# pierregab/VUB_Image_denoising

Measured on NVIDIA B200. Metric: denoised_mpix_per_s, higher is better.
Workload: dtype bf16

## Files before the change

vub_image_denoising_b200/csrc/common.cuh:

```cuda
#pragma once

#include <cuda.h>
#include <cuda_runtime.h>
#include <cuda_bf16.h>
#include <cuda_fp16.h>
#include <stdint.h>
#include <stdio.h>
#include <stdarg.h>

#include "../../include/b200dn.h"

namespace b200dn {

void set_error(const char* fmt, ...);
int cuda_fail(cudaError_t e, const char* what);

#define B200DN_CHECK_ARG(cond, ...)                      \
  do {                                                   \
    if (!(cond)) {                                       \
      ::b200dn::set_error(__VA_ARGS__);                  \
      return B200DN_E_ARG;                               \
    }                                                    \
  } while (0)

// ... 59 lines not shown
      : "r"(bar), "r"(parity)
      : "memory");
  return ok;
}
__device__ __forceinline__ bool elect_one() {
  uint32_t pred;
  asm volatile(
      "{\n\t"
      ".reg .pred p;\n\t"
      "elect.sync _|p, 0xffffffff;\n\t"
      "selp.b32 %0, 1, 0, p;\n\t"
      "}"
      : "=r"(pred));
  return pred != 0;
}
#ifndef B200DN_WATCHDOG_CYCLES
#define B200DN_WATCHDOG_CYCLES (4000000000ll)
#endif
__device__ __forceinline__ void mbar_wait(uint32_t bar, uint32_t parity) {
  if (mbar_try_wait(bar, parity)) return;
  const long long t0 = clock64();
  uint32_t spins = 0;
  while (!mbar_try_wait(bar, parity)) {
    if ((++spins & 0x3ff) == 0 && (clock64() - t0) > B200DN_WATCHDOG_CYCLES) {
      printf("b200dn: mbarrier watchdog (block %d thread %d bar 0x%x parity %u)\n", (int)blockIdx.x,
             (int)threadIdx.x, bar, parity);
      __trap();
    }
  }
}

__device__ __forceinline__ void griddep_wait() { asm volatile("griddepcontrol.wait;" ::: "memory"); }
__device__ __forceinline__ void griddep_launch_dependents() { asm volatile("griddepcontrol.launch_dependents;" ::: "memory"); }

__device__ __forceinline__ uint32_t cluster_ctarank() {
  uint32_t r;
  asm volatile("mov.u32 %0, %%cluster_ctarank;" : "=r"(r));
  return r;
}
__device__ __forceinline__ uint32_t mapa_shared(uint32_t addr, uint32_t rank) {
  uint32_t r;
  asm volatile("mapa.shared::cluster.u32 %0, %1, %2;" : "=r"(r) : "r"(addr), "r"(rank));
  return r;
}
__device__ __forceinline__ void mbar_arrive_cluster(uint32_t cluster_addr) {
  asm volatile("mbarrier.arrive.relaxed.cluster.shared::cluster.b64 _, [%0];" ::"r"(cluster_addr) : "memory");
}
__device__ __forceinline__ void mbar_arrive_remote(uint32_t cluster_addr) {
  asm volatile("mbarrier.arrive.shared::cluster.b64 _, [%0];" ::"r"(cluster_addr) : "memory");
}
__device__ __forceinline__ void cluster_sync_all() {
  asm volatile("barrier.cluster.arrive.release.aligned;\n\tbarrier.cluster.wait.acquire.aligned;" ::: "memory");
}

__device__ __forceinline__ void fence_proxy_async_smem() {
  asm volatile("fence.proxy.async.shared::cta;" ::: "memory");
}

__device__ __forceinline__ void tma_prefetch_desc(const void* desc) {
  asm volatile("prefetch.tensormap [%0];" ::"l"(reinterpret_cast<uint64_t>(desc)) : "memory");
}
__device__ __forceinline__ void tma_load_3d(uint32_t dst, const void* desc, uint32_t bar, int c0, int c1, int c2) {
  asm volatile(
      "cp.async.bulk.tensor.3d.shared::cluster.global.mbarrier::complete_tx::bytes [%0], [%1, {%3, %4, %5}], [%2];"
      ::"r"(dst), "l"(reinterpret_cast<uint64_t>(desc)), "r"(bar), "r"(c0), "r"(c1), "r"(c2)
      : "memory");
}
__device__ __forceinline__ void tma_load_4d(uint32_t dst, const void* desc, uint32_t bar, int c0, int c1, int c2,
                                            int c3) {
  asm volatile(
      "cp.async.bulk.tensor.4d.shared::cluster.global.mbarrier::complete_tx::bytes [%0], [%1, {%3, %4, %5, %6}], [%2];"
      ::"r"(dst), "l"(reinterpret_cast<uint64_t>(desc)), "r"(bar), "r"(c0), "r"(c1), "r"(c2), "r"(c3)
      : "memory");
}
__device__ __forceinline__ void tma_load_5d(uint32_t dst, const void* desc, uint32_t bar, int c0, int c1, int c2,
                                            int c3, int c4) {
  asm volatile(
      "cp.async.bulk.tensor.5d.shared::cluster.global.mbarrier::complete_tx::bytes [%0], [%1, {%3, %4, %5, %6, %7}], "
      "[%2];"
      ::"r"(dst), "l"(reinterpret_cast<uint64_t>(desc)), "r"(bar), "r"(c0), "r"(c1), "r"(c2), "r"(c3), "r"(c4)
      : "memory");
}

__device__ __forceinline__ void tma_load_3d_2sm(uint32_t dst, const void* desc, uint32_t bar, int c0, int c1, int c2) {
  asm volatile(
      "cp.async.bulk.tensor.3d.cta_group::2.shared::cluster.global.mbarrier::complete_tx::bytes [%0], [%1, {%3, %4, %5}], "
      "[%2];"
      ::"r"(dst), "l"(reinterpret_cast<uint64_t>(desc)), "r"(bar), "r"(c0), "r"(c1), "r"(c2)
      : "memory");
}
__device__ __forceinline__ void tma_load_4d_2sm(uint32_t dst, const void* desc, uint32_t bar, int c0, int c1, int c2,
                                                int c3) {
  asm volatile(
      "cp.async.bulk.tensor.4d.cta_group::2.shared::cluster.global.mbarrier::complete_tx::bytes [%0], [%1, {%3, %4, %5, "
      "%6}], [%2];"
      ::"r"(dst), "l"(reinterpret_cast<uint64_t>(desc)), "r"(bar), "r"(c0), "r"(c1), "r"(c2), "r"(c3)
      : "memory");
}

__device__ __forceinline__ void tmem_alloc(uint32_t dst_smem, uint32_t ncols) {
  asm volatile("tcgen05.alloc.cta_group::1.sync.aligned.shared::cta.b32 [%0], %1;" ::"r"(dst_smem), "r"(ncols)
               : "memory");
}
__device__ __forceinline__ void tmem_relinquish() {
  asm volatile("tcgen05.relinquish_alloc_permit.cta_group::1.sync.aligned;" ::: "memory");
}
__device__ __forceinline__ void tmem_dealloc(uint32_t taddr, uint32_t ncols) {
  asm volatile("tcgen05.dealloc.cta_group::1.sync.aligned.b32 %0, %1;" ::"r"(taddr), "r"(ncols) : "memory");
}
__device__ __forceinline__ void tc_fence_before() { asm volatile("tcgen05.fence::before_thread_sync;" ::: "memory"); }
__device__ __forceinline__ void tc_fence_after() { asm volatile("tcgen05.fence::after_thread_sync;" ::: "memory"); }
__device__ __forceinline__ void tmem_ld_wait() { asm volatile("tcgen05.wait::ld.sync.aligned;" ::: "memory"); }

__device__ __forceinline__ void umma_f16(uint32_t tmem_d, uint64_t desc_a, uint64_t desc_b, uint32_t idesc,
                                         uint32_t accumulate) {
  asm volatile(
      "{\n\t"
      ".reg .pred p;\n\t"
      "setp.ne.b32 p, %4, 0;\n\t"
      "tcgen05.mma.cta_group::1.kind::f16 [%0], %1, %2, %3, p;\n\t"
      "}"
      ::"r"(tmem_d), "l"(desc_a), "l"(desc_b), "r"(idesc), "r"(accumulate)
      : "memory");
}
__device__ __forceinline__ void umma_commit(uint32_t bar) {
  asm volatile("tcgen05.commit.cta_group::1.mbarrier::arrive::one.shared::cluster.b64 [%0];" ::"r"(bar) : "memory");
}

__device__ __forceinline__ void tmem_alloc_2cta(uint32_t dst_smem, uint32_t ncols) {
  asm volatile("tcgen05.alloc.cta_group::2.sync.aligned.shared::cta.b32 [%0], %1;" ::"r"(dst_smem), "r"(ncols)
               : "memory");
}
__device__ __forceinline__ void tmem_relinquish_2cta() {
  asm volatile("tcgen05.relinquish_alloc_permit.cta_group::2.sync.aligned;" ::: "memory");
}
__device__ __forceinline__ void tmem_dealloc_2cta(uint32_t taddr, uint32_t ncols) {
  asm volatile("tcgen05.dealloc.cta_group::2.sync.aligned.b32 %0, %1;" ::"r"(taddr), "r"(ncols) : "memory");
}
__device__ __forceinline__ void umma_f16_2cta(uint32_t tmem_d, uint64_t desc_a, uint64_t desc_b, uint32_t idesc,
                                              uint32_t accumulate) {
  asm volatile(
      "{\n\t"
      ".reg .pred p;\n\t"
      "setp.ne.b32 p, %4, 0;\n\t"
      "tcgen05.mma.cta_group::2.kind::f16 [%0], %1, %2, %3, p;\n\t"
      "}"
      ::"r"(tmem_d), "l"(desc_a), "l"(desc_b), "r"(idesc), "r"(accumulate)
      : "memory");
}
__device__ __forceinline__ void umma_commit_2cta(uint32_t bar, uint16_t cta_mask) {
  asm volatile("tcgen05.commit.cta_group::2.mbarrier::arrive::one.shared::cluster.multicast::cluster.b64 [%0], %1;"
               ::"r"(bar), "h"(cta_mask)
               : "memory");
}

__device__ __forceinline__ void tmem_ld16(uint32_t taddr, uint32_t (&r)[16]) {
  asm volatile(
      "tcgen05.ld.sync.aligned.32x32b.x16.b32 "
      "{%0, %1, %2, %3, %4, %5, %6, %7, %8, %9, %10, %11, %12, %13, %14, %15}, [%16];"
      : "=r"(r[0]), "=r"(r[1]), "=r"(r[2]), "=r"(r[3]), "=r"(r[4]), "=r"(r[5]), "=r"(r[6]), "=r"(r[7]), "=r"(r[8]),
        "=r"(r[9]), "=r"(r[10]), "=r"(r[11]), "=r"(r[12]), "=r"(r[13]), "=r"(r[14]), "=r"(r[15])
      : "r"(taddr)
      : "memory");
}

__device__ __forceinline__ uint64_t make_sw128_desc(uint32_t smem_addr, uint32_t sbo_bytes) {
// ... 33 lines not shown
```

vub_image_denoising_b200/csrc/igemm_common.cuh:

```cuda
#pragma once
#include "common.cuh"

#include <cudaTypedefs.h>

namespace b200dn {
namespace igemm {

constexpr int BLOCK_M = 128;
constexpr int BLOCK_K = 64;
constexpr int A_BYTES = BLOCK_M * BLOCK_K * 2;
constexpr int MAX_N = 256;
constexpr int NUM_THREADS = 256;
constexpr int EPI_THREADS = 128;
constexpr int MAX_STAGES = 8;

struct __align__(64) KParams {
  CUtensorMap tmA0, tmA1, tmW;
  int taps;
  int B, H, W;
  int n_cblk, last_k16;
  int cout, block_n;
  int mt;
  int n_tiles_per_group, num_n_tiles;
  int tiles_x, tiles_y, num_tiles;
  int n_pairs, pair_a[3], pair_w[3];
  int wgroups;
  int fmt;
  int num_stages, stage_bytes, tmem_cols;
  int slab_w, slab_bytes, num_slabs;
  int slab_tx;
  int wres, n_wplanes;
  int w_taps;
  int cta2, num_m_tiles;
  int epi_staged;
  int up_fold;
  const float* bias;
  const float* slope;
  int out_kind;
  void* out0;
  void* out1;
  int out_ctot, out_coff;
  const void* res0;
  const void* res1;
  int res_ctot;
  float* out_nchw;
  const float* res_nchw;
  int res_bmod;
  int* sat_flag;
#ifdef B200DN_TIMELINE
  unsigned long long* tl;
#endif
};

enum { TL_ENTRY = 0, TL_SETUP = 1, TL_DEP = 2, TL_MMA0 = 3, TL_MMA_END = 4, TL_ACC0 = 5, TL_EPI_END = 6, TL_EXIT = 7, TL_SM = 8 };
#ifdef B200DN_TIMELINE
__device__ __forceinline__ unsigned long long tl_now() {
  unsigned long long t;
  asm volatile("mov.u64 %0, %%globaltimer;" : "=l"(t));
  return t;
}
#define TL_MARK(p, slot)                                          \
  do {                                                            \
    if ((p).tl != nullptr && blockIdx.x == 0) (p).tl[slot] = tl_now(); \
  } while (0)
#define TL_MARK_ONCE(p, slot, flag)                               \
  do {                                                            \
    if (!(flag)) {                                                \
      (flag) = true;                                              \
      TL_MARK(p, slot);                                           \
    }                                                             \
  } while (0)
#else
#define TL_MARK(p, slot) do {} while (0)
#define TL_MARK_ONCE(p, slot, flag) do {} while (0)
#endif

struct TileCoord {
  int b, y0, x0, grp, n0;
};

__device__ __forceinline__ TileCoord decode_tile(int tile, int num_n_tiles, int n_tiles_per_group, int block_n,
                                                 int tiles_x, int tiles_y, int tile_w, int tile_h) {
  TileCoord t;
  const int m_tile = tile / num_n_tiles;
  const int nt = tile - m_tile * num_n_tiles;
  t.grp = nt / n_tiles_per_group;
  t.n0 = (nt - t.grp * n_tiles_per_group) * block_n;
  const int per_img = tiles_x * tiles_y;
  t.b = m_tile / per_img;
  const int r = m_tile - t.b * per_img;
  const int ty = r / tiles_x;
  t.y0 = ty * tile_h;
  t.x0 = (r - ty * tiles_x) * tile_w;
  return t;
}

struct TileWalker {
  int nt, tx, ty, b;
  int s_nt, s_tx, s_ty, s_b;
  int num_n_tiles, tiles_x, tiles_y;
  __device__ __forceinline__ void init(int tile, int stride, int num_n_tiles_, int tiles_x_, int tiles_y_) {
    num_n_tiles = num_n_tiles_, tiles_x = tiles_x_, tiles_y = tiles_y_;
    int m = tile / num_n_tiles;
    nt = tile - m * num_n_tiles;
    int q = m / tiles_x;
    tx = m - q * tiles_x;
    b = q / tiles_y;
    ty = q - b * tiles_y;
    m = stride / num_n_tiles;
    s_nt = stride - m * num_n_tiles;
    q = m / tiles_x;
    s_tx = m - q * tiles_x;
    s_b = q / tiles_y;
    s_ty = q - s_b * tiles_y;
  }
  __device__ __forceinline__ void next() {
    nt += s_nt;
    int c = nt >= num_n_tiles ? 1 : 0;
// ... 470 lines not shown
```

vub_image_denoising_b200/csrc/igemm_sm100.cu:

```cuda
#include "igemm_common.cuh"
#ifdef B200DN_TIMELINE
#include <mutex>
#include <string>
#include <vector>
#endif

#include <mutex>
#include <new>
#include <stdlib.h>
#include <string.h>

#ifndef B200DN_DEFAULT_CONV3X3_IMPL
#define B200DN_DEFAULT_CONV3X3_IMPL 2
#endif

namespace b200dn {

using namespace igemm;

namespace {

constexpr int TILE_W = 16;
constexpr int TILE_H = 8;
constexpr int RING_BYTES = 176 * 1024;
constexpr int TAP_STAGING_BYTES = 32 * 1024;
constexpr int DATA_BYTES = RING_BYTES + TAP_STAGING_BYTES;
constexpr int SMEM_BYTES = 1024 + DATA_BYTES + 256 + 2 * 2 * MAX_N * 4;

template <int MODE, int MT>
constexpr int epi_groups() { return (MODE == 2 && MT == 1) ? 2 : 1; }

template <int MODE, int MT>
__global__ void __launch_bounds__(NUM_THREADS + EPI_THREADS * (epi_groups<MODE, MT>() - 1), 1)
igemm_kernel(const __grid_constant__ KParams p) {
  constexpr int EG = epi_groups<MODE, MT>();
  extern __shared__ uint8_t smem_raw[];
  const uint32_t raw_u32 = smem_u32(smem_raw);
  const uint32_t smem_base = (raw_u32 + 1023u) & ~1023u;
  uint8_t* smem_gen = smem_raw + (smem_base - raw_u32);
  const uint32_t bars = smem_base + DATA_BYTES;
  if (threadIdx.x == 0) TL_MARK(p, TL_ENTRY);
  uint32_t* tmem_ptr_s = reinterpret_cast<uint32_t*>(smem_gen + DATA_BYTES + 160);
  float* epi_bias = reinterpret_cast<float*>(smem_gen + DATA_BYTES + 256);
  float* epi_slope = epi_bias + 2 * MAX_N;

  const int warp = (threadIdx.x >> 5) ^ 4;
  const int lane = threadIdx.x & 31;

  if (warp == 0 && lane == 0) {
    tma_prefetch_desc(&p.tmA0);
    tma_prefetch_desc(&p.tmW);
    if (p.n_pairs > 1) tma_prefetch_desc(&p.tmA1);
  }
  if (warp == 1 && lane == 0) {
    for (int s = 0; s < MAX_STAGES; ++s) {
      mbar_init(bars + s * 8, 2);
      mbar_init(bars + 64 + s * 8, MT);
    }
    for (int a = 0; a < 2; ++a) {
      mbar_init(bars + 128 + a * 8, MT);
      mbar_init(bars + 144 + a * 8, (EPI_THREADS / 32) * EG);
    }
    mbar_fence_init();
  }
  if (warp == 2) {
    tmem_alloc(smem_u32(tmem_ptr_s), static_cast<uint32_t>(p.tmem_cols));
    tmem_relinquish();
  }
  tc_fence_before();
  __syncthreads();
  tc_fence_after();
  const uint32_t tmem_base = *tmem_ptr_s;
  if (threadIdx.x == 0) TL_MARK(p, TL_SETUP);
  griddep_launch_dependents();
  if (warp != 2) griddep_wait();
  if (threadIdx.x == 0) TL_MARK(p, TL_DEP);

  const int num_tiles = p.num_tiles, grid = gridDim.x;
  const int num_n_tiles = p.num_n_tiles, n_tiles_per_group = p.n_tiles_per_group, block_n = p.block_n;
  const int tiles_x = p.tiles_x, tiles_y = p.tiles_y;
  const int n_cblk = p.n_cblk, n_pairs = p.n_pairs, num_stages = p.num_stages, stage_bytes = p.stage_bytes;
  constexpr int KY = MODE == 0 ? 3 : MODE == 1 ? 2 : 1;
  constexpr int KX = KY;
  constexpr uint32_t W_OFF = MT * A_BYTES;
  constexpr int STW = TILE_W * MT;

  if (warp == 0) {
    int stage = 0;
    uint32_t phase = 0;
    const int pa0 = p.pair_a[0], pa1 = p.pair_a[1], pa2 = p.pair_a[2];
    TileWalker tw_;
    tw_.init(blockIdx.x, grid, num_n_tiles, tiles_x, tiles_y);
    for (int tile = blockIdx.x; tile < num_tiles; tile += grid, tw_.next()) {
      const TileCoord t = tw_.coord_groups(block_n, n_tiles_per_group, STW, TILE_H);
      for (int pair = 0; pair < n_pairs; ++pair) {
        const int pa = pair == 0 ? pa0 : pair == 1 ? pa1 : pa2;
        const CUtensorMap* tmA = pa ? &p.tmA1 : &p.tmA0;
#pragma unroll
        for (int ky = 0; ky < KY; ++ky) {
#pragma unroll
          for (int kx = 0; kx < KX; ++kx) {
            for (int cb = 0; cb < n_cblk; ++cb) {
              mbar_wait(bars + 64 + stage * 8, phase ^ 1u);
              if (elect_one()) {
                const uint32_t full = bars + stage * 8;
                const uint32_t a_dst = smem_base + stage * stage_bytes;
                mbar_arrive_expect_tx(full, MT * A_BYTES);
#pragma unroll
                for (int j = 0; j < MT; ++j) {
                  const int xj = t.x0 + j * TILE_W;
                  if (MODE == 0)
                    tma_load_4d(a_dst + j * A_BYTES, tmA, full, cb * BLOCK_K, xj + kx - 1, t.y0 + ky - 1, t.b);
                  else if (MODE == 1)
// ... 22 lines not shown
    tw_.init(blockIdx.x, grid, num_n_tiles, tiles_x, tiles_y);
    for (int tile = blockIdx.x; tile < num_tiles; tile += grid, tw_.next()) {
      const TileCoord t = tw_.coord_groups(block_n, n_tiles_per_group, STW, TILE_H);
      for (int pair = 0; pair < n_pairs; ++pair) {
        const int wbase = pair == 0 ? pw0 : pair == 1 ? pw1 : pw2;
#pragma unroll
        for (int tap = 0; tap < KY * KX; ++tap) {
          const int wslice = wbase + (MODE == 2 ? t.grp : tap);
          for (int cb = 0; cb < n_cblk; ++cb) {
            mbar_wait(bars + 64 + stage * 8, phase ^ 1u);
            if (elect_one()) {
              const uint32_t full = bars + stage * 8;
              mbar_arrive_expect_tx(full, w_bytes);
              tma_load_3d(smem_base + stage * stage_bytes + W_OFF, &p.tmW, full, cb * BLOCK_K, t.n0, wslice);
            }
            __syncwarp();
            if (++stage == num_stages) {
              stage = 0;
              phase ^= 1u;
            }
          }
        }
      }
    }
  } else if (warp == 1 || (warp == 3 && MT == 2)) {
    const int j = warp == 1 ? 0 : 1;
    const uint32_t idesc = make_idesc_f16(static_cast<uint32_t>(p.fmt), static_cast<uint32_t>(block_n));
    const int k_iters = n_pairs * p.taps * n_cblk;
    const int last_k16 = p.last_k16;
    const uint32_t a_off = static_cast<uint32_t>(j * A_BYTES);
    int stage = 0;
    uint32_t phase = 0;
    int local_tile = 0;
    uint32_t ready = 0;
    for (int tile = blockIdx.x; tile < num_tiles; tile += grid, ++local_tile) {
      const int acc = local_tile & 1;
      const uint32_t acc_phase = (local_tile >> 1) & 1;
      mbar_wait(bars + 144 + acc * 8, acc_phase ^ 1u);
      const uint32_t d = tmem_base + static_cast<uint32_t>((acc * MT + j) * block_n);
      uint32_t accumulate = 0;
      int cb = 0;
      for (int kit = 0; kit < k_iters; ++kit) {
        if (!ready) mbar_wait(bars + stage * 8, phase);
        tc_fence_after();
        const uint32_t s_addr = smem_base + stage * stage_bytes;
        const uint32_t empty_bar = bars + 64 + stage * 8;
        const bool full_block = (cb != n_cblk - 1) || (last_k16 == BLOCK_K / 16);
        if (++stage == num_stages) {
          stage = 0;
          phase ^= 1u;
        }
        ready = mbar_test_wait(bars + stage * 8, phase);
        if (elect_one()) {
          const uint64_t adesc = make_sw128_desc(s_addr + a_off, 1024);
          const uint64_t bdesc = make_sw128_desc(s_addr + W_OFF, 1024);
          if (full_block) {
            umma_f16(d, adesc, bdesc, idesc, accumulate);
            umma_f16(d, adesc + 2, bdesc + 2, idesc, 1u);
            umma_f16(d, adesc + 4, bdesc + 4, idesc, 1u);
            umma_f16(d, adesc + 6, bdesc + 6, idesc, 1u);
          } else {
            for (int k = 0; k < last_k16; ++k) umma_f16(d, adesc + 2 * k, bdesc + 2 * k, idesc, k == 0 ? accumulate : 1u);
          }
          umma_commit(empty_bar);
          if (kit == k_iters - 1) umma_commit(bars + 128 + acc * 8);
        }
        __syncwarp();
        accumulate = 1;
        if (++cb == n_cblk) cb = 0;
      }
    }
  } else if (warp >= 4) {
    const int we = warp & 3;
    const int eg = (EG == 2 && warp >= 8) ? 1 : 0;
    const int row = we * 32 + lane;
    const int th = row / TILE_W, tw = row - th * TILE_W;
    const int et = (threadIdx.x & (EPI_THREADS - 1)) + eg * EPI_THREADS;
    const EpiArgs ea = make_epi_args(p);
    const int H = p.H, W = p.W, cout = p.cout;
    const float* bias = p.bias;
    const float* slope = p.slope;
    const bool up = p.wgroups == 4 && MODE == 2;
    const bool staged = p.epi_staged;
    uint8_t* stg = smem_gen + RING_BYTES + (eg * 4 + we) * 4096;
    const int ncols = block_n / EG, col0 = eg * ncols;
    const bool one_n_tile = n_tiles_per_group == 1;
    if (one_n_tile) stage_bias_slope(epi_bias, epi_slope, bias, slope, 0, block_n, cout, et, EPI_THREADS * EG);
    int local_tile = 0;
    uint32_t satm = 0;
    TileWalker tw_;
    tw_.init(blockIdx.x, grid, num_n_tiles, tiles_x, tiles_y);
    for (int tile = blockIdx.x; tile < num_tiles; tile += grid, ++local_tile, tw_.next()) {
      const TileCoord t = tw_.coord_groups(block_n, n_tiles_per_group, STW, TILE_H);
      const int acc = local_tile & 1;
      const uint32_t acc_phase = (local_tile >> 1) & 1;
      float* bs = epi_bias + (one_n_tile ? 0 : acc * MAX_N);
      float* ss = epi_slope + (one_n_tile ? 0 : acc * MAX_N);
      if (!one_n_tile) stage_bias_slope(bs, ss, bias, slope, t.n0, block_n, cout, et, EPI_THREADS * EG);

      mbar_wait(bars + 128 + acc * 8, acc_phase);
      tc_fence_after();

#pragma unroll 1
      for (int j = 0; j < MT; ++j) {
        const int y = t.y0 + th, x = t.x0 + j * TILE_W + tw;
        const bool valid = (y < H) && (x < W);
        const int64_t res_pix = (static_cast<int64_t>(t.b) * H + y) * W + x;
        int64_t out_pix = res_pix;
        if (up) {
          const int ky = t.grp >> 1, kx = t.grp & 1;
          out_pix = (static_cast<int64_t>(t.b) * (2 * H) + (2 * y + ky)) * (2 * W) + (2 * x + kx);
        }
        const uint32_t taddr =
            tmem_base + (static_cast<uint32_t>(we * 32) << 16) + static_cast<uint32_t>((acc * MT + j) * block_n + col0);
        const uint32_t rel = j == MT - 1 ? bars + 144 + acc * 8 : 0u;
        if (MODE == 2 && p.up_fold) {
#pragma unroll 1
          for (int q = 0; q < 4 / EG; ++q) {
            const int ph = eg * (4 / EG) + q, ky = ph >> 1, kx = ph & 1;
            const uint32_t tq = taddr + static_cast<uint32_t>(q * cout);
            const uint32_t relq = q == 4 / EG - 1 ? rel : 0u;
            if (staged) {
              RowMap rm;
              rm.b = t.b, rm.y0 = t.y0, rm.x0 = t.x0 + j * TILE_W, rm.tw_shift = 4, rm.H = H, rm.W = W;
              rm.up = 1, rm.ky = ky, rm.kx = kx;
              epilogue_subtile_staged(ea, tq, cout, bs, ss, rm, we * 32, lane, 0, relq, stg, satm);
            } else {
              const int64_t op = (static_cast<int64_t>(t.b) * (2 * H) + (2 * y + ky)) * (2 * W) + (2 * x + kx);
              epilogue_subtile(ea, tq, cout, bs, ss, valid, t.b, y, x, op, res_pix, 0, relq, satm);
            }
          }
        } else if (staged) {
          RowMap rm;
          rm.b = t.b, rm.y0 = t.y0, rm.x0 = t.x0 + j * TILE_W, rm.tw_shift = 4, rm.H = H, rm.W = W;
          rm.up = up ? 1 : 0, rm.ky = t.grp >> 1, rm.kx = t.grp & 1;
          epilogue_subtile_staged(ea, taddr, ncols, bs + col0, ss + col0, rm, we * 32, lane, t.n0 + col0, rel, stg, satm);
        } else {
          epilogue_subtile(ea, taddr, ncols, bs + col0, ss + col0, valid, t.b, y, x, out_pix, res_pix, t.n0 + col0, rel, satm);
        }
      }
    }
    sat_report(ea.sat_flag, satm);
  }

  tc_fence_before();
  __syncthreads();
  if (warp == 2) {
    tc_fence_after();
    tmem_dealloc(tmem_base, static_cast<uint32_t>(p.tmem_cols));
  }
  if (threadIdx.x == 0) TL_MARK(p, TL_EXIT);
}

PFN_cuTensorMapEncodeTiled g_encode = nullptr;
std::once_flag g_encode_once;

int get_encoder() {
  std::call_once(g_encode_once, [] {
    void* fn = nullptr;
    cudaDriverEntryPointQueryResult q;
    if (cudaGetDriverEntryPoint("cuTensorMapEncodeTiled", &fn, cudaEnableDefault, &q) == cudaSuccess &&
        q == cudaDriverEntryPointSuccess)
      g_encode = reinterpret_cast<PFN_cuTensorMapEncodeTiled>(fn);
  });
  if (!g_encode) {
    set_error("cuTensorMapEncodeTiled entry point not available (no CUDA driver?)");
    return B200DN_E_CUDA;
  }
  return 0;
}

int encode(CUtensorMap* tm, CUtensorMapDataType dt, int rank, const void* base, const uint64_t* dims,
           const uint64_t* strides_bytes, const uint32_t* box, const char* what,
           CUtensorMapL2promotion promo = CU_TENSOR_MAP_L2_PROMOTION_L2_256B) {
  uint32_t estr[5] = {1, 1, 1, 1, 1};
  CUresult r = g_encode(tm, dt, static_cast<cuuint32_t>(rank), const_cast<void*>(base), dims, strides_bytes, box, estr,
                        CU_TENSOR_MAP_INTERLEAVE_NONE, CU_TENSOR_MAP_SWIZZLE_128B, promo,
                        CU_TENSOR_MAP_FLOAT_OOB_FILL_NONE);
  if (r != CUDA_SUCCESS) {
    set_error("cuTensorMapEncodeTiled(%s) failed with CUresult %d (rank %d dims %llu %llu %llu %llu %llu)", what,
              static_cast<int>(r), rank, (unsigned long long)dims[0], (unsigned long long)dims[1],
              (unsigned long long)(rank > 2 ? dims[2] : 0), (unsigned long long)(rank > 3 ? dims[3] : 0),
              (unsigned long long)(rank > 4 ? dims[4] : 0));
    return B200DN_E_CUDA;
  }
  return 0;
}

SmemOptIn g_smem_opt_in;

int default_conv3x3_impl() {
  static int impl = [] {
    const char* e = getenv("B200DN_CONV3X3_IMPL");
    if (e && !strcmp(e, "tap")) return 1;
    if (e && !strcmp(e, "slab")) return 2;
    return B200DN_DEFAULT_CONV3X3_IMPL;
  }();
  return impl;
}
int staged_mode() {
  static int mode = [] {
    const char* e = getenv("B200DN_EPI_STAGED");
    return e ? atoi(e) : 2;
  }();
  return mode;
}
bool wres_enabled() {
  static int on = [] {
    const char* e = getenv("B200DN_SLAB_WRES");
    return e ? atoi(e) : 1;
  }();
  return on != 0;
}
int cta2_mode() {
  static int mode = [] {
    const char* e = getenv("B200DN_CTA2");
    return e ? atoi(e) : 1;
  }();
  return mode;
}
int up_fold_enabled() {
  static int v = [] {
    const char* e = getenv("B200DN_UP_FOLD");
    return e ? atoi(e) : 1;
  }();
  return v;
}
int split_n_floor() {
  static int v = [] {
    const char* e = getenv("B200DN_SPLIT_N");
    const int x = e ? atoi(e) : 64;
    return x <= 0 ? 256 : x < 16 ? 16 : x;
  }();
  return v;
}
bool w_row_stages() {
  static int on = [] {
    const char* e = getenv("B200DN_W_ROW_STAGES");
    return e ? atoi(e) : 1;
  }();
  return on != 0;
}
int slab_pitch() {
  static int w = [] {
    const char* e = getenv("B200DN_SLAB_PITCH");
    const int v = e ? atoi(e) : 10;
    return v < 10 ? 10 : v > 16 ? 16 : v;
  }();
  return w;
}
CUtensorMapL2promotion a_l2_promotion() {
  static int v = [] {
    const char* e = getenv("B200DN_L2PROMO");
    return e ? atoi(e) : 3;
  }();
  return v == 0 ? CU_TENSOR_MAP_L2_PROMOTION_NONE : v == 1 ? CU_TENSOR_MAP_L2_PROMOTION_L2_64B
       : v == 2 ? CU_TENSOR_MAP_L2_PROMOTION_L2_128B : CU_TENSOR_MAP_L2_PROMOTION_L2_256B;
}

}

int igemm_configure(const b200dn_igemm_args& a, LaunchCfg* cfg, b200dn_igemm_plan_info* info, int sms_override) {
  B200DN_CHECK_ARG(a.mode >= 0 && a.mode <= 3, "igemm: bad mode %d", a.mode);
  B200DN_CHECK_ARG(a.prec >= 0 && a.prec <= 4, "igemm: bad prec %d", a.prec);
  B200DN_CHECK_ARG(a.B > 0 && a.H > 0 && a.W > 0 && a.cin > 0 && a.cout > 0, "igemm: non-positive dims");
  B200DN_CHECK_ARG(a.in[0] && a.wpacked && a.bias, "igemm: null input/weight/bias pointer");
  B200DN_CHECK_ARG(a.in_ctot % 8 == 0 && a.in_ctot >= a.cin, "igemm: in_ctot %d must be a multiple of 8 and >= cin %d",
                   a.in_ctot, a.cin);
  B200DN_CHECK_ARG(a.impl >= 0 && a.impl <= 3, "igemm: bad impl %d", a.impl);
  const bool two_a = (a.prec == B200DN_PREC_BF16X2 || a.prec == B200DN_PREC_BF16X3 || a.prec == B200DN_PREC_FP16X2);
  const bool two_w = (a.prec == B200DN_PREC_BF16X3);
  B200DN_CHECK_ARG(!two_a || a.in[1], "igemm: prec %d needs the lo activation plane in[1]", a.prec);
  if (a.mode == B200DN_MODE_DOWN2X2)
    B200DN_CHECK_ARG(a.H % 2 == 0 && a.W % 2 == 0, "igemm: DOWN2X2 needs even H, W (got %d x %d)", a.H, a.W);
  if (info == nullptr) {
    B200DN_CHECK_ARG(cfg != nullptr, "igemm: internal: no launch configuration to fill");
    if (int rc = require_sm100()) return rc;
    if (int rc = get_encoder()) return rc;
  } else {
    B200DN_CHECK_ARG(sms_override > 0, "igemm_plan: sm_count must be positive");
  }
  const int impl = a.impl ? a.impl : default_conv3x3_impl();
  const bool slab = a.mode == B200DN_MODE_CONV3X3 && impl >= 2;

  KParams p_local;
  KParams& p = cfg ? cfg->p : p_local;
  memset(&p, 0, sizeof(p));
  p.sat_flag = a.sat_flag;
  p.taps = a.mode == B200DN_MODE_CONV3X3 ? 9 : a.mode == B200DN_MODE_DOWN2X2 ? 4 : 1;
  p.wgroups = a.mode == B200DN_MODE_CONV3X3 ? 9 : a.mode == B200DN_MODE_CONV1X1 ? 1 : 4;
  const int n_groups = a.mode == B200DN_MODE_UP2X2 ? 4 : 1;
  if (a.mode == B200DN_MODE_DOWN2X2) {
    p.B = 1;
    p.H = a.B * (a.H / 2);
    p.W = a.W / 2;
  } else {
    p.B = a.B;
    p.H = a.H;
    p.W = a.W;
  }
  p.n_cblk = cdiv(a.cin, BLOCK_K);
  p.last_k16 = cdiv(a.cin - (p.n_cblk - 1) * BLOCK_K, 16);
  p.cout = a.cout;
  const int cin_pad = round_up(a.cin, BLOCK_K);
  const int cout_pad = round_up(a.cout, 16);
  int sms = info ? sms_override : device_sm_count();
  if (sms <= 0) return B200DN_E_CUDA;
  int block_n = a.block_n;
  const bool up_fold = a.mode == B200DN_MODE_UP2X2 && block_n == 0 && a.m_tiles != 2 && up_fold_enabled() &&
// ... 15 lines not shown
  p.n_tiles_per_group = up_fold ? 1 : cdiv(cout_pad, block_n);
  p.num_n_tiles = up_fold ? 1 : p.n_tiles_per_group * n_groups;
  const int tw1 = slab ? SLAB_TILE_W : TILE_W, th1 = slab ? SLAB_TILE_H : TILE_H;
  int mt = a.m_tiles;
  B200DN_CHECK_ARG(mt >= 0 && mt <= 2, "igemm: m_tiles %d invalid", mt);
  if (mt == 2) B200DN_CHECK_ARG(block_n <= 128, "igemm: m_tiles=2 needs block_n <= 128 (TMEM columns)");
  if (mt == 0) {
    const int64_t tiles2 = slab ? static_cast<int64_t>(p.B) * cdiv(p.W, tw1) * cdiv(p.H, 2 * th1) * p.num_n_tiles
                                : static_cast<int64_t>(p.B) * cdiv(p.W, 2 * tw1) * cdiv(p.H, th1) * p.num_n_tiles;
    mt = (block_n <= 128 && tiles2 >= 2 * sms) ? 2 : 1;
    if (a.mode == B200DN_MODE_UP2X2) mt = 1;
  }
  p.mt = mt;
  const int stw = slab ? tw1 : tw1 * mt, sth = slab ? th1 * mt : th1;
  p.tiles_x = cdiv(p.W, stw);
  p.tiles_y = cdiv(p.H, sth);
  p.num_m_tiles = p.B * p.tiles_x * p.tiles_y;
  p.num_tiles = p.num_m_tiles * p.num_n_tiles;
  p.fmt = (a.prec == B200DN_PREC_FP16 || a.prec == B200DN_PREC_FP16X2) ? 0 : 1;
  switch (a.prec) {
    case B200DN_PREC_BF16X2:
    case B200DN_PREC_FP16X2:
      p.n_pairs = 2;
      p.pair_w[0] = 0, p.pair_a[0] = 1;
      p.pair_w[1] = 0, p.pair_a[1] = 0;
      break;
    case B200DN_PREC_BF16X3:
      p.n_pairs = 3;
      p.pair_w[0] = 1, p.pair_a[0] = 0;
      p.pair_w[1] = 0, p.pair_a[1] = 1;
      p.pair_w[2] = 0, p.pair_a[2] = 0;
      break;
    default:
      p.n_pairs = 1;
      p.pair_w[0] = 0, p.pair_a[0] = 0;
  }
  if (slab) {
    p.slab_w = slab_pitch();
    p.slab_tx = p.slab_w * (SLAB_TILE_H * mt + 2) * 128;
    p.slab_bytes = round_up(p.slab_tx, 1024);
    p.n_wplanes = two_w ? 2 : 1;
    const int64_t w_all = static_cast<int64_t>(p.n_wplanes) * p.n_cblk * 9 * block_n * 128;
    const int pair_tiles0 = cdiv(p.num_m_tiles, 2) * p.num_n_tiles;
    const bool small_n_pairs = a.impl == 0 && cta2_mode() >= 1 && block_n >= 32 && block_n < 64 && a.cin >= 64 &&
                               pair_tiles0 >= sms / 2;
    p.wres = (impl != 3 && !small_n_pairs && p.num_n_tiles == 1 && block_n < 64 &&
              w_all <= SLAB_WRES_BYTES - 2 * p.slab_bytes && wres_enabled()) ? 1 : 0;
    const int pair_tiles = cdiv(p.num_m_tiles, 2) * p.num_n_tiles;
    const bool pairs_fit = pair_tiles >= sms / 2 || (cta2_mode() == 1 && p.num_tiles < sms && p.num_m_tiles >= 2);
    p.cta2 = (!p.wres && block_n >= 32 &&
              (impl == 3 || small_n_pairs || (a.impl == 0 && cta2_mode() >= 1 && block_n >= 64 && pairs_fit))) ? 1 : 0;
    if (p.cta2) p.num_tiles = pair_tiles;
    p.w_taps = 1;
    if (p.wres) {
      p.num_slabs = static_cast<int>((SLAB_WRES_BYTES - w_all) / p.slab_bytes);
      p.stage_bytes = block_n * 128;
      p.num_stages = 1;
    } else {
      p.w_taps = (block_n <= 64 && w_row_stages()) ? 3 : 1;
      p.stage_bytes = (p.cta2 ? block_n / 2 : block_n) * 128 * p.w_taps;
      int want = p.w_taps == 3 ? (p.cta2 ? 5 : 4) : block_n > 128 ? 4 : block_n > 64 ? 6 : 8;
      p.num_slabs = (SLAB_DATA_BYTES - want * p.stage_bytes) / p.slab_bytes;
      if (p.num_slabs < 2) p.num_slabs = 2;
      if (p.num_slabs > SLAB_MAX_SLABS) p.num_slabs = SLAB_MAX_SLABS;
      p.num_stages = (SLAB_DATA_BYTES - p.num_slabs * p.slab_bytes) / p.stage_bytes;
      if (p.num_stages > MAX_STAGES) p.num_stages = MAX_STAGES;
    }
    if (p.num_slabs > SLAB_MAX_SLABS) p.num_slabs = SLAB_MAX_SLABS;
  } else {
    p.stage_bytes = mt * A_BYTES + block_n * 128;
    p.num_stages = RING_BYTES / p.stage_bytes;
    if (p.num_stages > MAX_STAGES) p.num_stages = MAX_STAGES;
  }
  int cols = 32;
  while (cols < 2 * mt * block_n) cols <<= 1;
  p.tmem_cols = cols;

  p.bias = a.bias;
  p.slope = a.slope;
  p.out_kind = a.out_kind;
  const int epi_cols = up_fold ? a.cout : (a.mode == B200DN_MODE_UP2X2 && mt == 1) ? block_n / 2 : block_n;
  p.epi_staged = (a.out_kind == B200DN_OUT_NHWC16 && !two_a && epi_cols % 64 == 0 && a.cout % 64 == 0 &&
                  a.out_coff % 64 == 0 && a.out_ctot % 8 == 0 && (staged_mode() == 1 || (staged_mode() == 2 && mt == 1))) ? 1 : 0;
  if (a.out_kind == B200DN_OUT_NHWC16) {
    B200DN_CHECK_ARG(a.out[0], "igemm: null NHWC output");
    B200DN_CHECK_ARG(!two_a || a.out[1], "igemm: prec %d needs the lo output plane out[1]", a.prec);
    B200DN_CHECK_ARG(a.out_ctot % 8 == 0 && a.out_coff % 8 == 0 && a.cout % 8 == 0 &&
                         a.out_coff + a.cout <= a.out_ctot,
                     "igemm: NHWC output slice [%d,%d) of %d must be 8-channel aligned", a.out_coff,
                     a.out_coff + a.cout, a.out_ctot);
    p.out0 = a.out[0];
    p.out1 = two_a ? a.out[1] : nullptr;
    p.out_ctot = a.out_ctot;
    p.out_coff = a.out_coff;
    if (a.res[0]) {
      B200DN_CHECK_ARG(a.mode == B200DN_MODE_CONV3X3 || a.mode == B200DN_MODE_CONV1X1,
                       "igemm: NHWC residual only with stride-1 modes");
      B200DN_CHECK_ARG(a.res_ctot % 8 == 0 && a.res_ctot >= a.cout, "igemm: bad res_ctot %d", a.res_ctot);
      B200DN_CHECK_ARG(!two_a || a.res[1], "igemm: prec %d needs the lo residual plane", a.prec);
      p.res0 = a.res[0];
      p.res1 = two_a ? a.res[1] : nullptr;
      p.res_ctot = a.res_ctot;
    }
  } else if (a.out_kind == B200DN_OUT_NCHW32) {
    B200DN_CHECK_ARG(a.out_nchw, "igemm: null NCHW output");
    B200DN_CHECK_ARG(a.mode == B200DN_MODE_CONV3X3 || a.mode == B200DN_MODE_CONV1X1,
                     "igemm: NCHW output only with stride-1 modes");
    p.out_nchw = a.out_nchw;
    p.res_nchw = a.res_nchw;
    p.res_bmod = a.res_bmod > 0 ? a.res_bmod : a.B;
  } else {
    B200DN_CHECK_ARG(false, "igemm: bad out_kind %d", a.out_kind);
  }

  int grid = p.num_tiles < sms ? p.num_tiles : sms;
  if (a.max_ctas > 0 && grid > a.max_ctas) grid = a.max_ctas;
  int clusters = 0;
  if (slab && p.cta2) {
    clusters = p.num_tiles < sms / 2 ? p.num_tiles : sms / 2;
    if (a.max_ctas > 0 && clusters > (a.max_ctas + 1) / 2) clusters = (a.max_ctas + 1) / 2;
  }
  if (info != nullptr) {
    memset(info, 0, sizeof(*info));
    info->kernel = slab ? (p.cta2 ? 2 : 1) : 0;
    info->mt = mt, info->block_n = block_n, info->num_n_tiles = p.num_n_tiles, info->num_tiles = p.num_tiles;
    info->grid = (slab && p.cta2) ? 2 * clusters : grid;
    info->wres = p.wres, info->num_slabs = slab ? p.num_slabs : 0, info->slab_bytes = slab ? p.slab_bytes : 0;
    info->num_stages = p.num_stages, info->stage_bytes = p.stage_bytes, info->w_taps = slab ? p.w_taps : 1;
    info->tmem_cols = p.tmem_cols, info->epi_staged = p.epi_staged;
    if (slab) {
      const int w_bytes = p.wres ? p.n_wplanes * p.n_cblk * 9 * block_n * 128 : p.num_stages * p.stage_bytes;
      info->data_bytes_used = p.num_slabs * p.slab_bytes + w_bytes;
      info->data_bytes_budget = p.wres ? SLAB_WRES_BYTES : SLAB_DATA_BYTES;
    } else {
      info->data_bytes_used = p.num_stages * p.stage_bytes;
      info->data_bytes_budget = RING_BYTES;
    }
    return 0;
  }

  const CUtensorMapDataType dt = p.fmt ? CU_TENSOR_MAP_DATA_TYPE_BFLOAT16 : CU_TENSOR_MAP_DATA_TYPE_FLOAT16;
  const uint64_t ct = static_cast<uint64_t>(a.in_ctot);
  for (int pl = 0; pl < (two_a ? 2 : 1); ++pl) {
    CUtensorMap* tm = pl ? &p.tmA1 : &p.tmA0;
    B200DN_CHECK_ARG((reinterpret_cast<uintptr_t>(a.in[pl]) & 15) == 0, "igemm: input plane %d not 16-byte aligned", pl);
    if (a.mode == B200DN_MODE_DOWN2X2) {
      uint64_t dims[5] = {static_cast<uint64_t>(a.cin), 2, static_cast<uint64_t>(a.W / 2), 2,
                          static_cast<uint64_t>(a.B) * (a.H / 2)};
      uint64_t str[4] = {ct * 2, 2 * ct * 2, static_cast<uint64_t>(a.W) * ct * 2, 2 * static_cast<uint64_t>(a.W) * ct * 2};
      uint32_t box[5] = {BLOCK_K, 1, TILE_W, 1, TILE_H};
      if (int rc = encode(tm, dt, 5, a.in[pl], dims, str, box, "A/down", a_l2_promotion())) return rc;
    } else {
      uint64_t dims[4] = {static_cast<uint64_t>(a.cin), static_cast<uint64_t>(a.W), static_cast<uint64_t>(a.H),
                          static_cast<uint64_t>(a.B)};
      uint64_t str[3] = {ct * 2, static_cast<uint64_t>(a.W) * ct * 2,
                         static_cast<uint64_t>(a.H) * static_cast<uint64_t>(a.W) * ct * 2};
      uint32_t box[4] = {BLOCK_K, TILE_W, TILE_H, 1};
      if (slab) {
        box[1] = static_cast<uint32_t>(p.slab_w);
        box[2] = static_cast<uint32_t>(SLAB_TILE_H * mt + 2);
      }
      if (int rc = encode(tm, dt, 4, a.in[pl], dims, str, box, slab ? "A/slab" : "A", a_l2_promotion())) return rc;
    }
  }
  {
    B200DN_CHECK_ARG((reinterpret_cast<uintptr_t>(a.wpacked) & 15) == 0, "igemm: packed weights not 16-byte aligned");
    uint64_t dims[3] = {static_cast<uint64_t>(cin_pad), static_cast<uint64_t>(cout_pad),
                        static_cast<uint64_t>(p.wgroups) * (two_w ? 2 : 1)};
    uint64_t str[2] = {static_cast<uint64_t>(cin_pad) * 2, static_cast<uint64_t>(cin_pad) * cout_pad * 2};
    uint32_t box[3] = {BLOCK_K, static_cast<uint32_t>(p.cta2 ? block_n / 2 : block_n),
                       p.wres ? 9u : static_cast<uint32_t>(slab ? p.w_taps : 1)};
    if (up_fold) box[1] = static_cast<uint32_t>(a.cout), box[2] = 4;
    if (int rc = encode(&p.tmW, dt, 3, a.wpacked, dims, str, box, "W")) return rc;
  }

  cfg->kind = 0;
  cfg->cooperative = 0;
#ifdef B200DN_TIMELINE
  {
    char label[96];
    snprintf(label, sizeof(label), "%s %dx%dx%d cin %d cout %d N %d mt %d %s", a.mode == B200DN_MODE_CONV3X3 ? "conv3x3"
             : a.mode == B200DN_MODE_DOWN2X2 ? "down" : "up", a.B, a.H, a.W, a.cin, a.cout, block_n, mt,
             slab ? (p.cta2 ? "pairs" : p.wres ? "wres" : "slab") : "tap");
    p.tl = igemm::timeline_slots(label);
  }
#endif
  if (slab && p.cta2) return resolve_conv3x3_slab2(cfg, 2 * clusters);
  if (slab) return resolve_conv3x3_slab(cfg, grid);

  static const void* const kernels[6] = {
      reinterpret_cast<const void*>(igemm_kernel<0, 1>), reinterpret_cast<const void*>(igemm_kernel<0, 2>),
      reinterpret_cast<const void*>(igemm_kernel<1, 1>), reinterpret_cast<const void*>(igemm_kernel<1, 2>),
      reinterpret_cast<const void*>(igemm_kernel<2, 1>), reinterpret_cast<const void*>(igemm_kernel<2, 2>)};
  if (int rc = ensure_max_dyn_smem(g_smem_opt_in, kernels, 6, SMEM_BYTES, "cudaFuncSetAttribute(igemm_kernel, smem)"))
    return rc;
  const int mode_idx = a.mode == B200DN_MODE_CONV3X3 ? 0 : a.mode == B200DN_MODE_DOWN2X2 ? 1 : 2;
  cfg->kernel = kernels[mode_idx * 2 + (mt - 1)];
  cfg->grid = grid;
  cfg->threads = NUM_THREADS + ((mode_idx == 2 && mt == 1) ? EPI_THREADS : 0);
  cfg->smem = SMEM_BYTES;
  cfg->cluster = 1;
  return 0;
}

int igemm_launch_cfg(const LaunchCfg& cfg, cudaStream_t stream) {
  void* params = cfg.kind == 1   ? static_cast<void*>(const_cast<FusedParams*>(&cfg.f))
                 : cfg.kind == 2 ? static_cast<void*>(const_cast<ChainParams*>(&cfg.c))
                                 : static_cast<void*>(const_cast<KParams*>(&cfg.p));
  B200DN_CUDA(launch_pdl(cfg.kernel, cfg.grid, cfg.threads, static_cast<size_t>(cfg.smem), stream, params, cfg.cluster,
                         cfg.cooperative != 0));
  return 0;
}

namespace igemm {
#ifdef B200DN_TIMELINE
namespace {
constexpr int TL_MAX_LAUNCHES = 4096;
unsigned long long* g_tl_base = nullptr;
std::vector<std::string> g_tl_labels;
std::mutex g_tl_mutex;
}
unsigned long long* timeline_slots(const char* label) {
  std::lock_guard<std::mutex> lock(g_tl_mutex);
  if (g_tl_base == nullptr) {
    if (cudaMalloc(&g_tl_base, TL_MAX_LAUNCHES * 16 * sizeof(unsigned long long)) != cudaSuccess) return nullptr;
    cudaMemset(g_tl_base, 0, TL_MAX_LAUNCHES * 16 * sizeof(unsigned long long));
  }
  if (static_cast<int>(g_tl_labels.size()) >= TL_MAX_LAUNCHES) return nullptr;
  g_tl_labels.emplace_back(label);
  return g_tl_base + (g_tl_labels.size() - 1) * 16;
}
#endif
int get_tensor_map_encoder(PFN_encodeTiled* fn) {
  if (int rc = get_encoder()) return rc;
  *fn = g_encode;
  return 0;
}
}

}

#ifdef B200DN_TIMELINE
extern "C" int b200dn_debug_timeline_dump(const char* path) {
  using namespace b200dn::igemm;
  std::lock_guard<std::mutex> lock(g_tl_mutex);
  if (g_tl_base == nullptr) return -1;
  cudaDeviceSynchronize();
  const size_t n = g_tl_labels.size();
  std::vector<unsigned long long> h(n * 16);
  if (cudaMemcpy(h.data(), g_tl_base, n * 16 * sizeof(unsigned long long), cudaMemcpyDeviceToHost) != cudaSuccess) return -2;
  FILE* f = fopen(path, "w");
  if (!f) return -3;
  fprintf(f, "# launch entry setup dep mma0 mma_end acc0 epi_end exit sm | label   (ns, absolute %%globaltimer; 0 = not recorded)\n");
  for (size_t i = 0; i < n; ++i) {
    fprintf(f, "%zu", i);
    for (int k = 0; k < 9; ++k) fprintf(f, " %llu", h[i * 16 + k]);
    fprintf(f, " | %s\n", g_tl_labels[i].c_str());
// ... 167 lines not shown
```

Baseline: 55.62.

## Use TMA bulk tensor stores for up/down-sample conv epilogues

Adds an epilogue path for the 2x2 down- and up-sampling implicit-GEMM kernels. Each warp stages bias+PReLU results for a 64-channel subtile in swizzled shared memory, then writes them to the NHWC output with cp.async.bulk.tensor stores, using 3D and 5D output tensor maps. The intent is to replace per-thread global stores with asynchronous bulk stores that overlap with the next subtile. In exchange it adds a wait on the staging buffer before each reuse, a restriction to 64-channel-aligned single-plane outputs, and a dependence on TMA boundary clipping for partial tiles.

```diff
diff --git a/vub_image_denoising_b200/csrc/common.cuh b/vub_image_denoising_b200/csrc/common.cuh
--- a/vub_image_denoising_b200/csrc/common.cuh
+++ b/vub_image_denoising_b200/csrc/common.cuh
@@ -165,6 +165,23 @@
       : "memory");
 }
 
+__device__ __forceinline__ void tma_store_3d(const void* desc, uint32_t src, int c0, int c1, int c2) {
+  asm volatile("cp.async.bulk.tensor.3d.global.shared::cta.bulk_group [%0, {%2, %3, %4}], [%1];"
+               ::"l"(reinterpret_cast<uint64_t>(desc)), "r"(src), "r"(c0), "r"(c1), "r"(c2)
+               : "memory");
+}
+__device__ __forceinline__ void tma_store_5d(const void* desc, uint32_t src, int c0, int c1, int c2, int c3, int c4) {
+  asm volatile("cp.async.bulk.tensor.5d.global.shared::cta.bulk_group [%0, {%2, %3, %4, %5, %6}], [%1];"
+               ::"l"(reinterpret_cast<uint64_t>(desc)), "r"(src), "r"(c0), "r"(c1), "r"(c2), "r"(c3), "r"(c4)
+               : "memory");
+}
+__device__ __forceinline__ void bulk_commit_group() { asm volatile("cp.async.bulk.commit_group;" ::: "memory"); }
+template <int N>
+__device__ __forceinline__ void bulk_wait_group_read() {
+  asm volatile("cp.async.bulk.wait_group.read %0;" ::"n"(N) : "memory");
+}
+__device__ __forceinline__ void bulk_wait_group_all() { asm volatile("cp.async.bulk.wait_group 0;" ::: "memory"); }
+
 __device__ __forceinline__ void tma_load_3d_2sm(uint32_t dst, const void* desc, uint32_t bar, int c0, int c1, int c2) {
   asm volatile(
       "cp.async.bulk.tensor.3d.cta_group::2.shared::cluster.global.mbarrier::complete_tx::bytes [%0], [%1, {%3, %4, %5}], "
diff --git a/vub_image_denoising_b200/csrc/igemm_common.cuh b/vub_image_denoising_b200/csrc/igemm_common.cuh
--- a/vub_image_denoising_b200/csrc/igemm_common.cuh
+++ b/vub_image_denoising_b200/csrc/igemm_common.cuh
@@ -16,6 +16,7 @@
 
 struct __align__(64) KParams {
   CUtensorMap tmA0, tmA1, tmW;
+  CUtensorMap tmO;
   int taps;
   int B, H, W;
   int n_cblk, last_k16;
@@ -34,6 +35,7 @@
   int cta2, num_m_tiles;
   int epi_staged;
   int up_fold;
+  int tma_store;
   const float* bias;
   const float* slope;
   int out_kind;
diff --git a/vub_image_denoising_b200/csrc/igemm_sm100.cu b/vub_image_denoising_b200/csrc/igemm_sm100.cu
--- a/vub_image_denoising_b200/csrc/igemm_sm100.cu
+++ b/vub_image_denoising_b200/csrc/igemm_sm100.cu
@@ -29,6 +29,67 @@
 
 template <int MODE, int MT>
 constexpr int epi_groups() { return (MODE == 2 && MT == 1) ? 2 : 1; }
+
+__device__ __forceinline__ void epilogue_subtile_tma(const EpiArgs& e, const CUtensorMap* tmO, bool up, uint32_t taddr,
+                                                     int ncols, const float* bs, const float* ss, int ch0, int kx,
+                                                     int x, int ky, int y, bool store, uint32_t release_bar,
+                                                     uint8_t* stg, uint32_t& satm) {
+  const uint32_t lane = threadIdx.x & 31;
+  const uint32_t stg_s = smem_u32(stg);
+  for (int c0 = 0; c0 < ncols; c0 += 64) {
+    uint32_t h[32];
+#pragma unroll
+    for (int q4 = 0; q4 < 4; ++q4) {
+      uint32_t r[16];
+      tmem_ld16(taddr + c0 + 16 * q4, r);
+      tmem_ld_wait();
+      if (release_bar != 0 && c0 + 64 >= ncols && q4 == 3) {
+        tc_fence_before();
+        __syncwarp();
+        if (lane == 0) mbar_arrive(release_bar);
+      }
+      float v[16];
+      const float4* b4 = reinterpret_cast<const float4*>(bs + c0 + 16 * q4);
+      const float4* s4 = reinterpret_cast<const float4*>(ss + c0 + 16 * q4);
+#pragma unroll
+      for (int q = 0; q < 4; ++q) {
+        const float4 bb = b4[q];
+        const float4 sl = s4[q];
+        float a;
+        a = __uint_as_float(r[4 * q + 0]) + bb.x;
+        v[4 * q + 0] = a > 0.f ? a : a * sl.x;
+        a = __uint_as_float(r[4 * q + 1]) + bb.y;
+        v[4 * q + 1] = a > 0.f ? a : a * sl.y;
+        a = __uint_as_float(r[4 * q + 2]) + bb.z;
+        v[4 * q + 2] = a > 0.f ? a : a * sl.z;
+        a = __uint_as_float(r[4 * q + 3]) + bb.w;
+        v[4 * q + 3] = a > 0.f ? a : a * sl.w;
+      }
+#pragma unroll
+      for (int j = 0; j < 8; ++j)
+        h[8 * q4 + j] = e.is_bf16 ? pack2<true>(v[2 * j], v[2 * j + 1]) : pack2<false>(v[2 * j], v[2 * j + 1]);
+      if (e.sat_flag != nullptr) {
+#pragma unroll
+        for (int j = 0; j < 8; ++j) satm = sat_track(satm, h[8 * q4 + j]);
+      }
+    }
+    if (lane == 0) bulk_wait_group_read<0>();
+    __syncwarp();
+#pragma unroll
+    for (int k = 0; k < 8; ++k)
+      *reinterpret_cast<uint4*>(stg + lane * 128 + ((k ^ (lane & 7)) << 4)) =
+          make_uint4(h[4 * k], h[4 * k + 1], h[4 * k + 2], h[4 * k + 3]);
+    fence_proxy_async_smem();
+    __syncwarp();
+    if (lane == 0 && store && ch0 + c0 < e.cout) {
+      if (up)
+        tma_store_5d(tmO, stg_s, ch0 + c0, kx, x, ky, y);
+      else
+        tma_store_3d(tmO, stg_s, ch0 + c0, x, y);
+      bulk_commit_group();
+    }
+  }
+}
 
 template <int MODE, int MT>
 __global__ void __launch_bounds__(NUM_THREADS + EPI_THREADS * (epi_groups<MODE, MT>() - 1), 1)
@@ -217,6 +278,8 @@
     const float* slope = p.slope;
     const bool up = p.wgroups == 4 && MODE == 2;
     const bool staged = p.epi_staged;
+    const bool tma = MODE != 0 && p.tma_store;
+    if (tma && lane == 0) tma_prefetch_desc(&p.tmO);
     uint8_t* stg = smem_gen + RING_BYTES + (eg * 4 + we) * 4096;
     const int ncols = block_n / EG, col0 = eg * ncols;
     const bool one_n_tile = n_tiles_per_group == 1;
@@ -249,7 +312,24 @@
         const uint32_t taddr =
             tmem_base + (static_cast<uint32_t>(we * 32) << 16) + static_cast<uint32_t>((acc * MT + j) * block_n + col0);
         const uint32_t rel = j == MT - 1 ? bars + 144 + acc * 8 : 0u;
-        if (MODE == 2 && p.up_fold) {
+        if (tma) {
+          const int yw = t.y0 + 2 * we, xw = t.x0 + j * TILE_W;
+          const bool rows_in = yw < H;
+          if (MODE == 2 && p.up_fold) {
+#pragma unroll 1
+            for (int q = 0; q < 4 / EG; ++q) {
+              const int ph = eg * (4 / EG) + q;
+              epilogue_subtile_tma(ea, &p.tmO, true, taddr + static_cast<uint32_t>(q * cout), cout, bs, ss, 0, ph & 1,
+                                   xw, ph >> 1, t.b * H + yw, rows_in, q == 4 / EG - 1 ? rel : 0u, stg, satm);
+            }
+          } else if (MODE == 2) {
+            epilogue_subtile_tma(ea, &p.tmO, true, taddr, ncols, bs + col0, ss + col0, t.n0 + col0, t.grp & 1, xw,
+                                 t.grp >> 1, t.b * H + yw, rows_in, rel, stg, satm);
+          } else {
+            epilogue_subtile_tma(ea, &p.tmO, false, taddr, ncols, bs + col0, ss + col0, t.n0 + col0, 0, xw, 0, yw,
+                                 rows_in, rel, stg, satm);
+          }
+        } else if (MODE == 2 && p.up_fold) {
 #pragma unroll 1
           for (int q = 0; q < 4 / EG; ++q) {
             const int ph = eg * (4 / EG) + q, ky = ph >> 1, kx = ph & 1;
@@ -276,6 +356,7 @@
       }
     }
     sat_report(ea.sat_flag, satm);
+    if (tma && lane == 0) bulk_wait_group_all();
   }
 
   tc_fence_before();
@@ -360,6 +441,10 @@
     return e ? atoi(e) : 1;
   }();
   return v;
+}
+bool updown_tma_store_enabled() {
+  const char* e = getenv("B200DN_UPDOWN_TMA_STORE");
+  return e ? atoi(e) != 0 : true;
 }
 int split_n_floor() {
   static int v = [] {
@@ -541,6 +626,9 @@
   const int epi_cols = up_fold ? a.cout : (a.mode == B200DN_MODE_UP2X2 && mt == 1) ? block_n / 2 : block_n;
   p.epi_staged = (a.out_kind == B200DN_OUT_NHWC16 && !two_a && epi_cols % 64 == 0 && a.cout % 64 == 0 &&
                   a.out_coff % 64 == 0 && a.out_ctot % 8 == 0 && (staged_mode() == 1 || (staged_mode() == 2 && mt == 1))) ? 1 : 0;
+  p.tma_store = ((a.mode == B200DN_MODE_DOWN2X2 || a.mode == B200DN_MODE_UP2X2) && a.out_kind == B200DN_OUT_NHWC16 &&
+                 !two_a && a.cout % 64 == 0 && epi_cols % 64 == 0 && (a.mode != B200DN_MODE_UP2X2 || a.H % 2 == 0) &&
+                 updown_tma_store_enabled()) ? 1 : 0;
   if (a.out_kind == B200DN_OUT_NHWC16) {
     B200DN_CHECK_ARG(a.out[0], "igemm: null NHWC output");
     B200DN_CHECK_ARG(!two_a || a.out[1], "igemm: prec %d needs the lo output plane out[1]", a.prec);
@@ -632,6 +720,24 @@
     if (up_fold) box[1] = static_cast<uint32_t>(a.cout), box[2] = 4;
     if (int rc = encode(&p.tmW, dt, 3, a.wpacked, dims, str, box, "W")) return rc;
   }
+  if (p.tma_store) {
+    B200DN_CHECK_ARG((reinterpret_cast<uintptr_t>(a.out[0]) & 15) == 0, "igemm: NHWC output not 16-byte aligned");
+    const void* base = static_cast<const uint16_t*>(a.out[0]) + a.out_coff;
+    const uint64_t cs = static_cast<uint64_t>(a.out_ctot) * 2;
+    if (a.mode == B200DN_MODE_DOWN2X2) {
+      const uint64_t wo = static_cast<uint64_t>(a.W / 2);
+      uint64_t dims[3] = {static_cast<uint64_t>(a.cout), wo, static_cast<uint64_t>(a.B) * (a.H / 2)};
+      uint64_t str[2] = {cs, wo * cs};
+      uint32_t box[3] = {64, TILE_W, 2};
+      if (int rc = encode(&p.tmO, dt, 3, base, dims, str, box, "O/down", CU_TENSOR_MAP_L2_PROMOTION_NONE)) return rc;
+    } else {
+      const uint64_t w = static_cast<uint64_t>(a.W);
+      uint64_t dims[5] = {static_cast<uint64_t>(a.cout), 2, w, 2, static_cast<uint64_t>(a.B) * a.H};
+      uint64_t str[4] = {cs, 2 * cs, 2 * w * cs, 4 * w * cs};
+      uint32_t box[5] = {64, 1, TILE_W, 1, 2};
+      if (int rc = encode(&p.tmO, dt, 5, base, dims, str, box, "O/up", CU_TENSOR_MAP_L2_PROMOTION_NONE)) return rc;
+    }
+  }
 
   cfg->kind = 0;
   cfg->cooperative = 0;
```

Result: no change. 55.78 (median of 6 runs) (+0.3%).
